# MLo7Ghinsan/GOOFER

Measured on AMD Instinct MI355X. Metric: resynth_frames_per_sec, higher is better.
Workload: dtype f32; 1 GPU; BASELINE config 3: 1024 notes/GPU x ~1.1 s, sr 44100, n_fft 1024, hop 256 (5.8 ms); per-note flags fa30fb-20fc10fd-10fw50fst40fsta20fstb-20fstc10fstd-10V80B20U-30 / fa-30fb20fc-10fd10fw-50fst-40fsta-20fstb20fstc-10fstd10V80B20U-30; one step = goofer_render_batch = goofer_assemble_batch + goofer_synth_batch (SillySampler.resample + gf.synthesize + V/B/U mix) from .goofy features and host-made plans; frames_per_gpu=194560, samples_per_gpu=49674240, sub_batches_per_gpu=1

## Files before the change

goofer_amd/csrc/api.hip:

```cpp
#include <math.h>
#include <stdarg.h>
#include <stdlib.h>

#include <algorithm>
#include <vector>

#include "common.h"
#include "launchers.h"

int goofer_fail(goofer_ctx *ctx, int code, const char *fmt, ...)
{
    if (ctx) {
        va_list ap;
        va_start(ap, fmt);
        vsnprintf(ctx->err, sizeof(ctx->err), fmt, ap);
        va_end(ap);
    }
    return code;
}

static goofer_ctx::kernel_state *kstate_of(goofer_ctx *ctx, const void *fn)
{
    for (int i = 0; i < ctx->n_kstate; ++i)
        if (ctx->kstate[i].fn == fn) return &ctx->kstate[i];
// ... 127 lines not shown
}

extern "C" {

const char *goofer_version(void) { return "goofer_hip 0.1 (gfx950)"; }

int goofer_create(int device_id, goofer_ctx **out)
{
    if (!out) return GOOFER_EINVAL;
    *out = nullptr;
    int count = 0;
    if (hipGetDeviceCount(&count) != hipSuccess || device_id < 0 || device_id >= count) return GOOFER_EHIP;
    if (hipSetDevice(device_id) != hipSuccess) return GOOFER_EHIP;
    goofer_ctx *c = new goofer_ctx();
    c->device = device_id;
    if (hipMalloc((void **)&c->ovf_flag, 64) != hipSuccess || hipMemset(c->ovf_flag, 0, 64) != hipSuccess) {
        delete c;
        return GOOFER_EHIP;
    }
    *out = c;
    return GOOFER_OK;
}

void goofer_destroy(goofer_ctx *ctx)
{
    if (!ctx) return;
    (void)hipSetDevice(ctx->device);
    (void)hipDeviceSynchronize();
    free_plan(ctx->plan);
    if (ctx->scratch) (void)hipFree(ctx->scratch);
    if (ctx->small) (void)hipFree(ctx->small);
// ... 218 lines not shown
    if (!ctx->ovf_flag) return GOOFER_OK;
    int32_t v = 0;
    HIP_TRY(ctx, hipMemcpy(&v, ctx->ovf_flag, sizeof(v), hipMemcpyDeviceToHost));
    if (v != 0) {
        HIP_TRY(ctx, hipMemset(ctx->ovf_flag, 0, sizeof(v)));
        return goofer_fail(ctx, GOOFER_EINVAL, "note %d of a batch since the last check has more pulse onsets than n / 2 + 16 (f0 above "
                           "sr / 2?): the pulses beyond its onset slots were dropped (the 'sg' layer's trackers have n + 16)", v - 1);
    }
    return GOOFER_OK;
}

int goofer_counter(goofer_ctx *ctx, const char *name, int64_t *value)
{
    if (!ctx || !name || !value) return GOOFER_EINVAL;
    int which = !strcmp(name, "pulse_fallback_notes") ? 1 : (!strcmp(name, "pulse_scanned_notes") ? 2 : -1);
    if (which < 0) return goofer_fail(ctx, GOOFER_EINVAL, "unknown counter %s", name);
    HIP_TRY(ctx, hipDeviceSynchronize());
    int32_t v = 0;
    HIP_TRY(ctx, hipMemcpy(&v, ctx->ovf_flag + which, sizeof(v), hipMemcpyDeviceToHost));
    *value = (int64_t)(uint32_t)v;
    return GOOFER_OK;
}

int64_t goofer_debug_fetch(goofer_ctx *ctx, int which, void *host_out, int64_t capacity_bytes)
{
    if (!ctx || which < 0 || which >= 16 || !ctx->dbg_ptr[which]) return GOOFER_EINVAL;
    if (int rc = goofer_check(ctx)) return rc;
    size_t nb = ctx->dbg_bytes[which] < (size_t)capacity_bytes ? ctx->dbg_bytes[which] : (size_t)capacity_bytes;
    if (hipMemcpy(host_out, ctx->dbg_ptr[which], nb, hipMemcpyDeviceToHost) != hipSuccess) return GOOFER_EHIP;
    return (int64_t)ctx->dbg_bytes[which];
}

// ... 73 lines not shown
    if (ctx && ctx->prof_stems) return PROF_NAMES_STEMS[stage];
    return (ctx && ctx->ola_fused) ? PROF_NAMES_OLA[stage] : PROF_NAMES[stage];
}

int goofer_set_option(goofer_ctx *ctx, const char *name, int value)
{
    if (!ctx || !name) return GOOFER_EINVAL;
    if (!strcmp(name, "fused_ola")) { ctx->ola_fused = value != 0; return GOOFER_OK; }
    if (!strcmp(name, "overlap")) { ctx->overlap = value != 0; return GOOFER_OK; }
    if (!strcmp(name, "stems")) { ctx->stems = value != 0; return GOOFER_OK; }
    if (!strcmp(name, "prof_only")) { ctx->prof_only = value < 0 || value >= PROF_STAGES ? -1 : value; return GOOFER_OK; }
    if (!strcmp(name, "skip_zero")) { ctx->skip_zero = value != 0; return GOOFER_OK; }
    if (!strcmp(name, "td_blur")) { ctx->td_blur = value != 0; return GOOFER_OK; }
    if (!strcmp(name, "pulse_scan")) { ctx->pulse_scan = value < 0 ? 0 : (value > 2 ? 2 : value); return GOOFER_OK; }
    if (!strcmp(name, "sa_fast")) { ctx->sa_fast = value != 0; return GOOFER_OK; }
    if (!strcmp(name, "value_f64")) { ctx->value_f64 = value != 0; return GOOFER_OK; }
    return goofer_fail(ctx, GOOFER_EINVAL, "unknown option %s", name);
}

int goofer_sizeof(int which)
{
    switch (which) {
    case 0: return (int)sizeof(goofer_note_params);
    case 1: return (int)sizeof(goofer_batch);
    case 2: return (int)sizeof(goofer_note_plan);
    case 3: return (int)sizeof(goofer_assembly);
    case 4: return (int)sizeof(goofer_onepole_job);
    case 5: return (int)sizeof(goofer_post_note);
    case 6: return (int)sizeof(goofer_post);
    case 7: return (int)sizeof(goofer_plan_request);
// ... 266 lines not shown
    if (!mask || !sample_off || !out || n_notes <= 0) return goofer_fail(ctx, GOOFER_EINVAL, "null argument");
    hipStream_t st = (hipStream_t)stream;
    std::vector<double> taps;
    int radius;
    gauss_taps_host(std::max(1.0, (double)sigma / 4.0), taps, radius);
    if (radius > 2048) return goofer_fail(ctx, GOOFER_EINVAL, "transition sigma too large");
    const size_t n_short = (size_t)(total_samples / 4 + n_notes + 16);
    int rc = grow_block(ctx, &ctx->small, &ctx->small_bytes, (taps.size() + 16 + n_short + 2 * (size_t)n_notes + 16) * sizeof(double),
                        "small block");
    if (rc) return rc;
    double *d_taps = (double *)ctx->small, *short_s = d_taps + taps.size() + 16, *steps = short_s + n_short;
    HIP_TRY(ctx, hipMemcpyAsync(d_taps, taps.data(), taps.size() * sizeof(double), hipMemcpyHostToDevice, st));
    HIP_TRY(ctx, hipStreamSynchronize(st));
    double acc = 0.0;
    for (double tv : taps) acc += tv * 1.0;
    if ((rc = launch_mask_short(ctx, mask, sample_off, n_notes, total_samples, d_taps, radius, acc, short_s, st))) return rc;
    return launch_mask_upsample(ctx, short_s, sample_off, n_notes, total_samples, steps, fast_interp != 0, out, st);
}

int goofer_normal_fill(goofer_ctx *ctx, uint64_t seed, const goofer_note_params *params, const int64_t *sample_off, int n_notes,
                       int64_t total_samples, int stream_tag, const unsigned char *note_on, const double *growl_scale, double *out,
                       void *stream)
{
    if (!ctx) return GOOFER_EINVAL;
    if (!params || !sample_off || !out) return goofer_fail(ctx, GOOFER_EINVAL, "goofer_normal_fill: null pointer");
    if (n_notes < 0 || total_samples < 0)
        return goofer_fail(ctx, GOOFER_EINVAL, "goofer_normal_fill: negative count (%d notes, %lld samples)", n_notes, (long long)total_samples);
    if (stream_tag < 0 || stream_tag > 4) return goofer_fail(ctx, GOOFER_EINVAL, "goofer_normal_fill: stream tag %d outside 0..4", stream_tag);
    if ((uintptr_t)out & 15) return goofer_fail(ctx, GOOFER_EINVAL, "goofer_normal_fill: out must be 16-byte aligned");
    return launch_normal_fill(ctx, seed, params, sample_off, n_notes, total_samples, stream_tag, note_on, growl_scale, out, (hipStream_t)stream);
}
// ... 86 lines not shown
```

goofer_amd/csrc/assemble.hip:

```cpp
#include <hip/hip_fp16.h>

#include <type_traits>

#include "binops_core.h"
#include "launchers.h"

constexpr int A_ROWS = 4;
constexpr int ES_HALO = 64;

__device__ __forceinline__ float exp_split(float x)
{
    const float L2E = 0x1.715476p+0f, L2E_LO = 0x1.4ae0c0p-26f, LN2 = 0x1.62e430p-1f;
    const float hi = x * L2E;
    float lo = __builtin_fmaf(x, L2E, -hi);
    lo = __builtin_fmaf(x, L2E_LO, lo);
    const float r = __builtin_amdgcn_exp2f(hi);
    return __builtin_fmaf(r, lo * LN2, r);
}

template <bool V64, int CH>
__global__ __launch_bounds__(256) void k_env_edit(const goofer_assembly a, int64_t total_edit_rows, const int *__restrict__ row_note)
{
    using acc_t = std::conditional_t<V64, double, float>;
    extern __shared__ __align__(16) unsigned char smem[];
// ... 641 lines not shown
}

__constant__ double EXP2_C[12] = {2.5678435993488206e-11, 4.4455382718708116e-10, 7.054911620801123e-09, 1.01780860092397e-07,
                                         1.321548679014431e-06,  1.5252733804059841e-05, 0.0001540353039338161,  0.0013333558146428443,
                                         0.009618129107628477,   0.05550410866482158,    0.24022650695910072,    0.6931471805599453};
__device__ __forceinline__ double exp2_poly(double x)
{
    const double n = rint(x), f = x - n;
    double q = EXP2_C[0];
#pragma unroll
    for (int k = 1; k < 12; ++k) q = fma(q, f, EXP2_C[k]);
    q = fma(q, f, 1.0);
    return ldexp(q, (int)n);
}

__device__ __forceinline__ void sample_assemble_one(const goofer_assembly &a, const goofer_note_plan &p, int64_t g)
{
    const int i = (int)(g - p.out_sample_off);
    const float *m = a.mask_src + p.src_sample_off;
    const float rd_tail = __builtin_amdgcn_rcpf((float)p.tail_len);

    double mk;
    if (p.vel_active) {
        const double pos = i < p.pre_new ? (double)i / p.vel_factor : (double)(i - p.pre_new) + (double)p.n_pre;
        const int n1 = p.n_before_vel;
        int j = pos >= 2147483647.0 ? n1 - 1 : (int)floor(pos);
        if (j > n1 - 1) j = n1 - 1;
        if (j < 0) j = 0;
        if (j >= n1 - 1) {
            mk = mask_stage1(m, p, n1 - 1, rd_tail);
        } else {
// ... 24 lines not shown
        } else if (j > 0 && x0 > tsec) {
            --j;
            x1 = x0;
            x0 = (double)j * dt;
        }
        if (j >= p.n_bend - 1) {
            midi = bend[p.n_bend - 1];
        } else {
            const double y0 = bend[j], y1 = bend[j + 1];
            const double den = x1 - x0;
            const double rden = fma(fma(-den, rdt, 1.0), rdt, rdt);
            midi = tsec == x0 ? y0 : ((y1 - y0) * rden) * (tsec - x0) + y0;
        }
    }
    const double hz = 440.0 * exp2_poly(div_by(midi - 69.0, 12.0, 0.083333333333333329));
    a.mask_out[g] = (float)mk;
    double f0 = mk * hz;
    if (p.pd_on && a.bend_out) a.bend_out[g] = (float)(midi - p.pd_base);
    if (p.fry_dir != 0) {
        const double base_hz = p.fry_hz * (mk > 0.0 ? 1.0 : 0.0);
        if (i >= p.fry_const_lo && i < p.fry_const_hi) {
            f0 = base_hz;
        } else if (i >= p.fry_glide_lo && i < p.fry_glide_hi) {
            const int m = p.fry_glide_hi - p.fry_glide_lo, k = i - p.fry_glide_lo;
            const double w = p.fry_dir > 0 ? ramp_up(k, m) : ramp_down(k, m);
            f0 = (1.0 - w) * base_hz + w * f0;
        }
    }
    a.f0_out[g] = (float)f0;
    if (a.f0_mul_out) a.f0_mul_out[g] = (float)(f0 * a.f0_mul[g]);
}


template <int SA_SPT>
__device__ __forceinline__ void sample_assemble_fast(const goofer_assembly &a, const goofer_note_plan &p, int64_t g0, int64_t total_samples)
{
    const float *__restrict__ m = a.mask_src + p.src_sample_off;
    const double *__restrict__ bend = a.bend + p.bend_off;
    float *__restrict__ mask_out = a.mask_out;
    float *__restrict__ f0_out = a.f0_out;
    const int n_pre = p.n_pre, s_pre = p.s_pre, s_tail = p.s_tail, tail_len = p.tail_len, ylen1 = (int)p.ylen - 1, nb1 = p.n_bend - 1;
    const bool tile = tail_len < p.want_samples, rev = p.reverse != 0, fv = p.force_voiced != 0;
    const float rd_tail = __builtin_amdgcn_rcpf((float)tail_len);
    const double sr = (double)a.sr, rsr = 1.0 / sr;
    const double dt = p.tick_dt, t_last = (double)nb1 * dt, rdt = fast_rcp(dt);
    const int64_t nbase = p.out_sample_off;
    int midx[SA_SPT], ja[SA_SPT], jb[SA_SPT];
    double tsec[SA_SPT], x0[SA_SPT], x1[SA_SPT];
    bool live[SA_SPT];
#pragma unroll
// ... 26 lines not shown
#pragma unroll
    for (int u = 0; u < SA_SPT; ++u) {
        mv[u] = fv ? 1.0f : m[midx[u]];
        y0[u] = bend[ja[u]];
        y1[u] = bend[jb[u]];
    }
    float fo[SA_SPT];
#pragma unroll
    for (int u = 0; u < SA_SPT; ++u) {
        const double den = x1[u] - x0[u];
        const double rden = fma(fma(-den, rdt, 1.0), rdt, rdt);
        const double midi = (ja[u] == jb[u] || tsec[u] == x0[u]) ? y0[u] : ((y1[u] - y0[u]) * rden) * (tsec[u] - x0[u]) + y0[u];
        const double hz = 440.0 * exp2_poly(div_by(midi - 69.0, 12.0, 0.083333333333333329));
        fo[u] = (float)((double)mv[u] * hz);
    }
#pragma unroll
    for (int u = 0; u < SA_SPT; ++u) {
        const int64_t g = g0 + threadIdx.x + (int64_t)u * blockDim.x;
        if (live[u]) {
            mask_out[g] = mv[u];
            f0_out[g] = fo[u];
        }
    }
}

template <int SA_SPT>
__global__ __launch_bounds__(256) void k_sample_assemble(const goofer_assembly a, int64_t total_samples, int fast)
{
    __shared__ int s_pair[2];
    const int64_t g0 = (int64_t)blockIdx.x * (blockDim.x * SA_SPT);
    if (threadIdx.x < WAVE) {
        auto key = [&](int k) { return a.notes[k].out_sample_off; };
        int64_t gl = g0 + (int64_t)blockDim.x * SA_SPT - 1;
        if (gl > total_samples - 1) gl = total_samples - 1;
        const int lo = wave_find(a.n_notes, g0, (int)threadIdx.x, key);
        const int hi = wave_find(a.n_notes, gl, (int)threadIdx.x, key);
        if (threadIdx.x == 0) { s_pair[0] = lo; s_pair[1] = hi; }
    }
    __syncthreads();
    const int n_lo = __builtin_amdgcn_readfirstlane(s_pair[0]), n_hi = __builtin_amdgcn_readfirstlane(s_pair[1]);
    if (n_lo == n_hi) {
        const goofer_note_plan &p = a.notes[n_lo];
        if (fast && !p.vel_active && p.fry_dir == 0 && !(p.pd_on && a.bend_out) && !a.f0_mul_out && p.n_out < (1 << 21) && p.tail_len < (1 << 24) &&
            p.tail_len > 0 && p.n_bend >= 1) {
            sample_assemble_fast<SA_SPT>(a, p, g0, total_samples);
            return;
        }
#pragma unroll
        for (int u = 0; u < SA_SPT; ++u) {
            const int64_t g = g0 + threadIdx.x + (int64_t)u * blockDim.x;
            if (g < total_samples) sample_assemble_one(a, p, g);
        }
    } else {
        for (int u = 0; u < SA_SPT; ++u) {
            const int64_t g = g0 + threadIdx.x + (int64_t)u * blockDim.x;
            if (g >= total_samples) break;
            int note = n_lo;
            while (note + 1 < a.n_notes && a.notes[note + 1].out_sample_off <= g) ++note;
            sample_assemble_one(a, a.notes[note], g);
        }
    }
}

__global__ __launch_bounds__(256) void k_env_fry(const goofer_assembly a, int64_t total_out_rows, const int *__restrict__ row_note, int hop)
{
    extern __shared__ __align__(16) unsigned char smem[];
    const int B = a.n_bins;
    const int wave = threadIdx.x >> 6, lane = threadIdx.x & 63;
    const int64_t orow = (int64_t)blockIdx.x * A_ROWS + wave;
    if (orow >= total_out_rows) return;
    const int note = row_note[orow];
    const goofer_note_plan p = a.notes[note];
    if (p.fry_a >= p.fry_b || p.n_out <= 0) return;
    const int64_t j = orow - p.env_off;
    int64_t c = j * hop + hop / 2;
// ... 46 lines not shown
        ctx->prof_asm_mask[ctx->prof_asm_steps] = 0;
    }
    auto mark = [&](int which, int edge, hipStream_t s) -> hipError_t {
        if (!pq || !(ctx->prof_only < 0 || ctx->prof_only == PROF_ASM0 + which)) return hipSuccess;
        if (edge) ctx->prof_asm_mask[ctx->prof_asm_steps] |= (unsigned char)(1u << which);
        return hipEventRecord(pq[2 * which + edge], s);
    };
    if (a->total_samples > 0) {
        const bool on_side = link.fork_early && ctx->ev_f0 && ctx->side && !a->any_fry;
        hipStream_t fst = on_side ? ctx->side : st;
        if (on_side) HIP_TRY(ctx, hipStreamWaitEvent(ctx->side, ctx->ev_entry, 0));
        constexpr int spt = 4;
        const dim3 sgrid((unsigned)((a->total_samples + 256 * spt - 1) / (256 * spt)));
        const int sa_fast = ctx->sa_fast ? 1 : 0;
        HIP_TRY(ctx, mark(2, 0, fst));
        hipLaunchKernelGGL(k_sample_assemble<spt>, sgrid, dim3(256), 0, fst, *a, a->total_samples, sa_fast);
        LAUNCH_CHECK(ctx);
        HIP_TRY(ctx, mark(2, 1, fst));
        if (link.fork_early && ctx->ev_f0) {
            HIP_TRY(ctx, hipEventRecord(ctx->ev_f0, fst));
            link.f0_ready = a->f0_out;
            link.f0_side = on_side;
        }
    }
    {
        const int64_t rows = std::max(a->total_edit_rows, a->total_out_rows);
        if (rows > 0) {
            hipLaunchKernelGGL(k_row_notes2, dim3((unsigned)((rows + 255) / 256)), dim3(256), 0, st, a->notes, a->n_notes, a->total_edit_rows,
                               a->total_out_rows, row_note_edit, row_note_out);
            LAUNCH_CHECK(ctx);
        }
// ... 74 lines not shown
```

goofer_amd/csrc/common.h:

```cpp
#pragma once

#include <hip/hip_runtime.h>
#include <stdint.h>
#include <stdio.h>
#include <string.h>

#include <vector>

#include "../../include/goofer_hip.h"

#define WAVE 64
#define PROF_STAGES 18
#define PROF_ASM0 15
#define PP_SPT 8
#define PULSE_TILE_INTS(samples) (4 * (((samples) + 256 * PP_SPT - 1) / (256 * PP_SPT)) + 64)
#define KN_K0 32
#define KN_DK 16
#define KN_KMAX 192
#define KN_CAND ((KN_KMAX - KN_K0) / KN_DK + 1)
#define KN_BINS_TOTAL (KN_CAND * KN_K0 + KN_DK * KN_CAND * (KN_CAND - 1) / 2)
#define PULSE_TAB_MAX 8192

struct lf_model {
    double ra = 0.02, rg = 1.7, rk = 0.8;
};
#define PULSE_PEAK_FLOATS (8193 + 1 + 6)

struct goofer_plan_t {
// ... 22 lines not shown
    float taps5_f[5] = {0}, taps175_f[15] = {0};
};

struct event_pool {
    int per_step;
    hipEvent_t *ev = nullptr;
    int steps = 0;
    hipEvent_t *step(int k) const { return ev + (size_t)k * per_step; }
};

struct render_link {
    bool fork_early = false;
    float *warp_dst = nullptr;
    const double *formants = nullptr;
    const goofer_note_params *params = nullptr;
    const float *f0_ready = nullptr;
    bool f0_side = false;
    bool warped = false;
};

struct goofer_ctx {
    int device = 0;
    char err[512] = {0};
    goofer_plan_t plan;
    void *scratch = nullptr;
    size_t scratch_bytes = 0;
    void *asm_scratch = nullptr;
    size_t asm_bytes = 0;
    void *small = nullptr;
    size_t small_bytes = 0;
    const void *dbg_ptr[16] = {nullptr};
    size_t dbg_bytes[16] = {0};
    bool overlap = true;
// ... 2 lines not shown
    hipEvent_t ev_entry = nullptr, ev_f0 = nullptr, ev_f0s = nullptr;
    int32_t *ovf_flag = nullptr;
    float *warp_rows = nullptr;
    size_t warp_rows_bytes = 0;
    event_pool prof_side{4};
    event_pool prof_main2{2};
    event_pool prof_asm{6};
    unsigned char prof_asm_mask[4096] = {0};
    int prof_asm_steps = 0;
    bool prof_side_used = false;
    bool ola_fused = true;
    bool stems = true;
    bool skip_zero = true;
    bool td_blur = true;
    bool prof_stems = false;
    bool sa_fast = true;
    bool value_f64 = false;
    int pulse_scan = 1;
    struct kernel_state {
        const void *fn;
        size_t lds;
        int waves;
        bool max_lds_set;
    } kstate[32] = {};
    int n_kstate = 0;
    bool prof_on = false;
    int prof_only = -1;
    int prof_steps = 0, prof_cap = 0;
    event_pool prof_ev{PROF_STAGES + 1};
    double *mask_taps = nullptr;
// ... 205 lines not shown
```

goofer_amd/csrc/launchers.h:

```cpp
#pragma once

#include "common.h"
#include "ragged.h"

struct onset_t;

int launch_gauss_rows64(goofer_ctx *ctx, const float *in, int ld, double *out, int ld64, int64_t rows, int n_bins, const double *d_taps,
                        int radius, hipStream_t st);
int launch_knot_error(goofer_ctx *ctx, const double *env2, int ld64, const int64_t *probe, int n_probe, int n_bins, const int *knot_bin,
                      int K, const int *lerp_idx, const float *w0, const float *w1, unsigned long long *err_bits, hipStream_t st);
int launch_knot_gather(goofer_ctx *ctx, const double *env2, int ld64, int64_t rows, const int *knot_bin, int K, uint16_t *knots,
                       hipStream_t st);
int launch_env_rows_fused(goofer_ctx *ctx, const float2 *S, int ldc, int64_t rows, int n_bins, const double *taps_env, int r_env,
                          const double *taps_fit, int r_fit, double *env_rows, int ld64, double *env2, int ld2, hipStream_t st);
int launch_knot_search(goofer_ctx *ctx, const double *env2, int ld2, const int64_t *probe_row, const int *probe_sig, int n_probe,
                       int n_bins, const int *knot_bin, const int *lerp_idx, const float *w0, const float *w1, unsigned long long *err_bits,
                       hipStream_t st);
int launch_knot_pick(goofer_ctx *ctx, const double *env2, int ld2, int64_t rows, const int *frame_sig, const int64_t *frame_off,
                     const int *knot_bin, const unsigned long long *err_bits, uint16_t *knots, int32_t *K_out, hipStream_t st);

size_t env_row_rec_bytes();
int launch_assemble(goofer_ctx *ctx, const goofer_assembly *a, int *row_note_edit, int *row_note_out, void *row_recs, render_link &link,
                    hipStream_t st);

// ... 92 lines not shown
                      const int *frame_note, const int64_t *frame_off, const int64_t *sample_off, int n_notes, const double *short_s,
                      double *steps, const goofer_note_params *params, float *harm, float *uv, float *bre, const unsigned char *frame_skip,
                      hipStream_t st);
int launch_frame_skip(goofer_ctx *ctx, const double *short_s, int64_t short_count, const int64_t *sample_off, const int64_t *frame_off,
                      const int *frame_note, int n_notes, int64_t total_frames, unsigned char *knot_eq, unsigned char *hop_flat,
                      unsigned char *frame_skip, hipStream_t st);
int launch_mask_upsample(goofer_ctx *ctx, const double *short_s, const int64_t *sample_off, int n_notes, int64_t total_samples,
                         double *steps, bool fast, float *out, hipStream_t st);
int launch_irfft_ola3(goofer_ctx *ctx, const float2 *S_h, const float2 *S_u, const float2 *S_b, int ldc, int64_t total_frames,
                      const int *frame_note, const int64_t *frame_off, const int64_t *sample_off, int n_notes, const float *note_mag,
                      const double *short_s, double *steps, const goofer_note_params *params, float *harm, float *uv, float *bre,
                      float *note_peak, hipStream_t st);
int launch_stem_peak(goofer_ctx *ctx, const float *harm, const float *uv, const float *bre, const int64_t *sample_off, int n_notes,
                     int64_t total, float *note_peak, hipStream_t st);
int launch_mask_short(goofer_ctx *ctx, const float *mask, const int64_t *sample_off, int n_notes, int64_t total_samples,
                      const double *d_taps, int radius, double tap_sum, double *short_s, hipStream_t st);
int launch_apply_gain(goofer_ctx *ctx, float *harm, float *uv, float *bre, float *rec, float *mix, const int64_t *sample_off, int n_notes,
                      int64_t total_samples, const goofer_note_params *params, const float *note_peak, bool write_stems, hipStream_t st);
int launch_ola3_gains(goofer_ctx *ctx, const float *fr_h, const float *fr_u, const float *fr_b, const float *note_mag,
                      const double *short_s, const int64_t *sample_off, const int64_t *frame_off, int n_notes, int64_t total_samples,
                      const goofer_note_params *params, double *steps, float *harm, float *uv, float *bre, float *note_peak,
                      hipStream_t st);

bool stems_supported(const goofer_plan_t &p);
int launch_frame_picks(goofer_ctx *ctx, const int64_t *frame_off, const int *frame_note, int64_t F, const int64_t *sample_off,
                       const float *f0, const float *mask, float2 *picks, hipStream_t st);
int launch_noise_stems(goofer_ctx *ctx, const float *env, int ld, const int64_t *row_src, const float *phi, int64_t F,
                       const int *frame_note, const int64_t *frame_off, const int64_t *sample_off, const float2 *picks,
                       const goofer_note_params *params, uint64_t seed, bool preblurred, const double *short_s, const double *steps,
                       float *uv, float *bre, unsigned char *hopz, hipStream_t st);
int launch_harm_stem(goofer_ctx *ctx, const float *pulse, const float *env, const float *env_plain, bool have_formants, int ld,
// ... 6 lines not shown
```

goofer_amd/csrc/samples.hip:

```cpp
#include <type_traits>
#include "fft_core.h"

#include "samples_core.h"
#include "launchers.h"

#define MS_MAXWIN 1152
#define MS_TILE 1024

__global__ __launch_bounds__(256) void k_mask_short(const float *__restrict__ mask, const int64_t *__restrict__ sample_off,
                                                    int n_notes, int64_t total_short, const double *__restrict__ taps, int radius,
                                                    double *__restrict__ short_s, double tap_sum)
{
    extern __shared__ __align__(16) unsigned char smem[];
    double *s_taps = reinterpret_cast<double *>(smem);
    float *s_all = reinterpret_cast<float *>(s_taps + (2 * radius + 1));
    __shared__ int s_lo[2];
    for (int i = threadIdx.x; i < 2 * radius + 1; i += blockDim.x) s_taps[i] = taps[i];
    const int64_t g0 = (int64_t)blockIdx.x * MS_TILE;
    int64_t g1 = g0 + MS_TILE;
    if (g1 > total_short) g1 = total_short;
    if (threadIdx.x < WAVE) {
        auto key = [&](int k) { return short_base(sample_off, k); };
        const int a = wave_find(n_notes, g0, (int)threadIdx.x, key);
        const int b = wave_find(n_notes, g1 - 1, (int)threadIdx.x, key);
        if (threadIdx.x == 0) { s_lo[0] = a; s_lo[1] = b; }
    }
    __syncthreads();
    const int lane = threadIdx.x & 63, wv = threadIdx.x >> 6;
    const int n_lo = __builtin_amdgcn_readfirstlane(s_lo[0]), n_hi = __builtin_amdgcn_readfirstlane(s_lo[1]);

    if (2 * radius + MS_TILE <= 4 * MS_MAXWIN) {
        for (int note = n_lo; note <= n_hi; ++note) {
            const int64_t sb = short_base(sample_off, note);
            const int64_t base = sample_off[note], n = sample_off[note + 1] - base;
            const int64_t ns = (n + MASK_DS - 1) / MASK_DS;
            const int64_t s0 = g0 > sb ? g0 : sb, s1 = g1 < sb + ns ? g1 : sb + ns;
            if (s1 <= s0) continue;
            const int64_t q0 = s0 - sb;
            const int len = (int)(s1 - s0);
            const float *m = mask + base;
            if (note != n_lo) __syncthreads();
            for (int w = threadIdx.x; w < len + 2 * radius; w += blockDim.x) s_all[w] = m[MASK_DS * reflect_index(q0 - radius + w, ns)];
            __syncthreads();
            for (int c0 = wv * WAVE; c0 < len; c0 += 4 * WAVE) {
                const float *x0 = s_all + c0;
                const int cl = len - c0 < WAVE ? len - c0 : WAVE;
                const bool live = lane < cl;
                bool all0 = true, all1 = true;
                for (int w = lane; w < cl + 2 * radius; w += WAVE) {
                    const float v = x0[w];
                    all0 &= v == 0.0f;
                    all1 &= v == 1.0f;
                }
                double acc;
                if (__all(all0)) {
                    acc = 0.0;
                } else if (__all(all1)) {
                    acc = tap_sum;
                } else {
                    acc = 0.0;
                    const float *x = x0 + lane;
                    if (live)
                        for (int j = 0; j <= 2 * radius; ++j) acc += s_taps[j] * (double)x[j];
                }
                if (live) short_s[s0 + c0 + lane] = acc;
            }
        }
        return;
    }
    for (int64_t g = g0 + threadIdx.x; g < g1; g += blockDim.x) {
        int note = n_lo;
        while (note + 1 < n_notes && short_base(sample_off, note + 1) <= g) ++note;
        const int64_t q = g - short_base(sample_off, note);
        const int64_t base = sample_off[note], n = sample_off[note + 1] - base;
        const int64_t ns = (n + MASK_DS - 1) / MASK_DS;
        if (q >= ns) continue;
        const float *m = mask + base;
        double acc = 0.0;
// ... 840 lines not shown
{
    const sample_tile<> t(sample_off, n_notes, total);
    const int64_t g = t.g;
    const float pk = t.live ? fabsf((harm[g] + uv[g]) + bre[g]) : 0.f;
    const int note = t.live && !t.uniform() ? t.note(sample_off) : t.lo;
    note_reduce(t, note, t.live, pk, [](float a, float b) { return fmaxf(a, b); }, [&](int k, float m) { atomic_max_pos(note_peak + k, m); });
}

int launch_stem_peak(goofer_ctx *ctx, const float *harm, const float *uv, const float *bre, const int64_t *sample_off, int n_notes,
                     int64_t total, float *note_peak, hipStream_t st)
{
    return launch_per_sample(ctx, k_stem_peak, total, 256, 0, st, harm, uv, bre, sample_off, n_notes, total, note_peak);
}

int launch_mask_short(goofer_ctx *ctx, const float *mask, const int64_t *sample_off, int n_notes, int64_t total_samples,
                      const double *d_taps, int radius, double tap_sum, double *short_s, hipStream_t st)
{
    int64_t total_short = total_samples / MASK_DS + n_notes;
    if (total_short <= 0) return GOOFER_OK;
    hipLaunchKernelGGL(k_mask_short, dim3((unsigned)((total_short + MS_TILE - 1) / MS_TILE)), dim3(256),
                       sizeof(double) * (2 * radius + 1) + sizeof(float) * 4 * MS_MAXWIN, st, mask, sample_off, n_notes, total_short,
                       d_taps, radius, short_s, tap_sum);
    LAUNCH_CHECK(ctx);
    return GOOFER_OK;
}

int launch_apply_gain(goofer_ctx *ctx, float *harm, float *uv, float *bre, float *rec, float *mix, const int64_t *sample_off,
                      int n_notes, int64_t total_samples, const goofer_note_params *params, const float *note_peak, bool write_stems,
                      hipStream_t st)
{
    return launch_per_sample(ctx, k_apply_gain, total_samples, 256 * SPT, 0, st, harm, uv, bre, rec, mix, sample_off, n_notes, total_samples,
                             params, note_peak, write_stems ? 1 : 0);
}

int launch_ola3_gains(goofer_ctx *ctx, const float *fr_h, const float *fr_u, const float *fr_b, const float *note_mag,
                      const double *short_s, const int64_t *sample_off, const int64_t *frame_off, int n_notes, int64_t total_samples,
                      const goofer_note_params *params, double *steps, float *harm, float *uv, float *bre, float *note_peak,
// ... 10 lines not shown
```

goofer_amd/csrc/synth.hip:

```cpp
#include <algorithm>
#include <vector>

#include "common.h"
#include "launchers.h"
#include "samples_core.h"

__device__ __forceinline__ void frame_pick_and_row(int64_t f, int note, const int64_t *__restrict__ frame_off,
                                                   const int64_t *__restrict__ env_off, int64_t *__restrict__ row_src,
                                                   const int64_t *__restrict__ sample_off, const float *__restrict__ f0,
                                                   const float *__restrict__ mask, int hop, float2 *__restrict__ picks)
{
    int64_t t = f - frame_off[note];
    if (picks) {
        const int64_t base = sample_off[note], n = sample_off[note + 1] - base;
        float2 pv = make_float2(0.f, 0.f);
        if (n > 0) {
            int64_t at = t * hop;
            if (at >= n) at = ((n - 1) / hop) * hop;
            pv = make_float2(f0[base + at], mask[base + at]);
        }
        picks[f] = pv;
    }
    const int64_t rows = env_off[note + 1] - env_off[note];
    if (t > rows - 1) t = rows - 1;
// ... 205 lines not shown
};

struct synth_call {
    goofer_ctx *ctx;
    const goofer_batch *b;
    const render_link &link;
    const synth_route &r;
    synth_scratch &s;
    stage_clock &clk;
    hipStream_t st;
    int64_t F, N;
    int n;

    int mask_short() const
    {
        return launch_mask_short(ctx, b->mask, b->sample_off, n, N, ctx->mask_taps, ctx->mask_taps_radius, ctx->mask_taps_sum, s.short_s, st);
    }
    int late_picks() const
    {
        return r.picks_on ? GOOFER_OK : launch_frame_picks(ctx, b->frame_off, s.frame_note, F, b->sample_off, s.f0s, b->mask, s.picks, st);
    }
    int noise_walker() const
    {
        return launch_noise_stems(ctx, b->env_noise ? b->env_noise : b->env, b->ld, s.row_src, b->phi, F, s.frame_note, b->frame_off,
                                  b->sample_off, s.picks, b->params, b->seed, b->env_noise != nullptr, s.short_s, s.note_steps, b->uv,
                                  b->bre, s.hopz, st);
    }
    int noise_spectra() const
    {
        return launch_noise_spectra(ctx, s.S_uv, s.S_br, spec_stride(ctx->plan.n_bins), F, s.frame_note, b->frame_off, b->sample_off, s.f0s,
                                    b->mask, b->env_noise ? b->env_noise : b->env, b->phi, b->ld, b->params, b->seed, s.row_src,
// ... 89 lines not shown
            return rc;
        return clk.close();
    }
};

static int assemble_batch(goofer_ctx *ctx, const goofer_assembly *asmb, render_link &link, hipStream_t st)
{
    if (asmb->n_notes <= 0) return GOOFER_OK;
    if (asmb->ld < asmb->n_bins || asmb->max_K < 2 || asmb->max_K > 4096) return goofer_fail(ctx, GOOFER_EINVAL, "bad assembly geometry");
    if (asmb->n_bins > 1025) return goofer_fail(ctx, GOOFER_EINVAL, "the resampler's assembly takes n_fft <= 2048 (%d bins)", asmb->n_bins);
    if (asmb->any_fry && ctx->plan.hop <= 0) return goofer_fail(ctx, GOOFER_EINVAL, "the fry envelope warp needs goofer_plan first");
    goofer_assembly a = *asmb;
    int *map_edit;
    float *edit_rows;
    char *recs;
    int rc = carve_block(ctx, &ctx->asm_scratch, &ctx->asm_bytes, "assembly scratch", [&](arena &m) {
        map_edit = m.take<int>((size_t)(a.total_edit_rows + a.total_out_rows) + 64);
        edit_rows = m.take<float>(a.edit_rows ? 0 : (size_t)a.total_edit_rows * a.ld);
        recs = m.take<char>((size_t)a.total_out_rows * env_row_rec_bytes());
    });
    if (rc) return rc;
    if (!a.edit_rows) a.edit_rows = edit_rows;
    return launch_assemble(ctx, &a, map_edit, map_edit + a.total_edit_rows, recs, link, st);
}

static int synth_batch(goofer_ctx *ctx, const goofer_batch *b, render_link &link, hipStream_t st)
{
    const goofer_plan_t &p = ctx->plan;
    if (b->n_bins != p.n_bins || b->ld < p.n_bins) return goofer_fail(ctx, GOOFER_EINVAL, "batch geometry does not match the plan");
    if (b->n_notes <= 0 || b->total_samples <= 0) return GOOFER_OK;
    const int64_t F = b->total_frames, N = b->total_samples;
    const int n = b->n_notes;
    const synth_route r = synth_route_of(ctx, b, link);
    synth_scratch s;
    int rc = carve_scratch(ctx, [&](arena &a) { carve_synth(a, p, r, F, N, n, b->ld, s); });
    if (rc) return rc;
// ... 174 lines not shown
    if (ctx->overlap && asmb->f0_out == b->f0 && asmb->n_notes > 0) {
        if ((rc = ensure_side_stream(ctx))) return rc;
        HIP_TRY(ctx, hipEventRecord(ctx->ev_entry, st));
        link.fork_early = true;
    }
    if (synth_route_of(ctx, b, link).walkers && ctx->overlap && asmb->env_out == b->env && asmb->n_notes == b->n_notes &&
        asmb->total_out_rows == b->total_env_rows && asmb->ld == b->ld && !asmb->any_fry) {
        const size_t need = (size_t)b->total_env_rows * b->ld * sizeof(float);
        if (need > ctx->warp_rows_bytes &&
            (rc = grow_block(ctx, (void **)&ctx->warp_rows, &ctx->warp_rows_bytes, need + need / 4, "warped rows")))
            return rc;
        link.formants = b->formants;
        link.params = b->params;
        link.warp_dst = ctx->warp_rows;
    }
    rc = assemble_batch(ctx, asmb, link, st);
    if (!rc) rc = synth_batch(ctx, b, link, st);
    if (link.f0_side) (void)hipStreamWaitEvent(st, ctx->ev_f0, 0);
    return rc;
}

}
```

Measured before the change: 106.2 million frames/s.

## Emit per-tile mask flatness flags in sample assembly to skip mask_short staging

```diff
diff --git a/goofer_amd/csrc/api.hip b/goofer_amd/csrc/api.hip
--- a/goofer_amd/csrc/api.hip
+++ b/goofer_amd/csrc/api.hip
@@ -165,7 +165,7 @@
     if (hipSetDevice(device_id) != hipSuccess) return GOOFER_EHIP;
     goofer_ctx *c = new goofer_ctx();
     c->device = device_id;
-    if (hipMalloc((void **)&c->ovf_flag, 64) != hipSuccess || hipMemset(c->ovf_flag, 0, 64) != hipSuccess) {
+    if (hipMalloc((void **)&c->ovf_flag, OVF_WORDS * sizeof(int32_t)) != hipSuccess || hipMemset(c->ovf_flag, 0, OVF_WORDS * sizeof(int32_t)) != hipSuccess) {
         delete c;
         return GOOFER_EHIP;
     }
@@ -414,8 +414,18 @@
 {
     if (!ctx || !name || !value) return GOOFER_EINVAL;
     int which = !strcmp(name, "pulse_fallback_notes") ? 1 : (!strcmp(name, "pulse_scanned_notes") ? 2 : -1);
-    if (which < 0) return goofer_fail(ctx, GOOFER_EINVAL, "unknown counter %s", name);
+    const int mask_c = !strcmp(name, "mask_flag_segments") ? 0 : (!strcmp(name, "mask_staged_segments") ? 1 : -1);
+    if (which < 0 && mask_c < 0) return goofer_fail(ctx, GOOFER_EINVAL, "unknown counter %s", name);
     HIP_TRY(ctx, hipDeviceSynchronize());
+    if (mask_c >= 0) {
+        static_assert(OVF_WORDS <= 8192, "goofer_counter reads the words through a stack buffer");
+        int32_t w[OVF_WORDS];
+        HIP_TRY(ctx, hipMemcpy(w, ctx->ovf_flag, sizeof(w), hipMemcpyDeviceToHost));
+        int64_t sum = 0;
+        for (int sl = 0; sl < MASK_COUNTER_SLOTS; ++sl) sum += (int64_t)(uint32_t)w[MASK_COUNTERS + (2 * sl + mask_c) * MASK_COUNTER_STRIDE];
+        *value = sum;
+        return GOOFER_OK;
+    }
     int32_t v = 0;
     HIP_TRY(ctx, hipMemcpy(&v, ctx->ovf_flag + which, sizeof(v), hipMemcpyDeviceToHost));
     *value = (int64_t)(uint32_t)v;
@@ -519,6 +529,7 @@
     if (!strcmp(name, "td_blur")) { ctx->td_blur = value != 0; return GOOFER_OK; }
     if (!strcmp(name, "pulse_scan")) { ctx->pulse_scan = value < 0 ? 0 : (value > 2 ? 2 : value); return GOOFER_OK; }
     if (!strcmp(name, "sa_fast")) { ctx->sa_fast = value != 0; return GOOFER_OK; }
+    if (!strcmp(name, "mask_flags")) { ctx->mask_flags = value != 0; return GOOFER_OK; }
     if (!strcmp(name, "value_f64")) { ctx->value_f64 = value != 0; return GOOFER_OK; }
     return goofer_fail(ctx, GOOFER_EINVAL, "unknown option %s", name);
 }
@@ -815,7 +826,7 @@
     HIP_TRY(ctx, hipStreamSynchronize(st));
     double acc = 0.0;
     for (double tv : taps) acc += tv * 1.0;
-    if ((rc = launch_mask_short(ctx, mask, sample_off, n_notes, total_samples, d_taps, radius, acc, short_s, st))) return rc;
+    if ((rc = launch_mask_short(ctx, mask, sample_off, n_notes, total_samples, d_taps, radius, acc, short_s, nullptr, nullptr, st))) return rc;
     return launch_mask_upsample(ctx, short_s, sample_off, n_notes, total_samples, steps, fast_interp != 0, out, st);
 }
 
diff --git a/goofer_amd/csrc/assemble.hip b/goofer_amd/csrc/assemble.hip
--- a/goofer_amd/csrc/assemble.hip
+++ b/goofer_amd/csrc/assemble.hip
@@ -679,7 +679,7 @@
     return ldexp(q, (int)n);
 }
 
-__device__ __forceinline__ void sample_assemble_one(const goofer_assembly &a, const goofer_note_plan &p, int64_t g)
+__device__ __forceinline__ float sample_assemble_one(const goofer_assembly &a, const goofer_note_plan &p, int64_t g)
 {
     const int i = (int)(g - p.out_sample_off);
     const float *m = a.mask_src + p.src_sample_off;
@@ -734,7 +734,8 @@
         }
     }
     const double hz = 440.0 * exp2_poly(div_by(midi - 69.0, 12.0, 0.083333333333333329));
-    a.mask_out[g] = (float)mk;
+    const float mk_f = (float)mk;
+    a.mask_out[g] = mk_f;
     double f0 = mk * hz;
     if (p.pd_on && a.bend_out) a.bend_out[g] = (float)(midi - p.pd_base);
     if (p.fry_dir != 0) {
@@ -749,11 +750,21 @@
     }
     a.f0_out[g] = (float)f0;
     if (a.f0_mul_out) a.f0_mul_out[g] = (float)(f0 * a.f0_mul[g]);
-}
-
-
-template <int SA_SPT>
-__device__ __forceinline__ void sample_assemble_fast(const goofer_assembly &a, const goofer_note_plan &p, int64_t g0, int64_t total_samples)
+    return mk_f;
+}
+
+
+__device__ __forceinline__ unsigned mask_vote(float mk) { return (mk == 0.0f ? 0u : 1u) | (mk == 1.0f ? 0u : 2u); }
+
+struct sa_kernarg {
+    goofer_assembly a;
+    int64_t total_samples;
+    int fast;
+    unsigned char *tile_flags;
+};
+template <int SA_SPT, bool FLAGS>
+__device__ __forceinline__ void sample_assemble_fast(const goofer_assembly &a, const goofer_note_plan &p, int64_t g0, int64_t total_samples,
+                                                     unsigned &bad, unsigned char *&flag_dst)
 {
     const float *__restrict__ m = a.mask_src + p.src_sample_off;
     const double *__restrict__ bend = a.bend + p.bend_off;
@@ -810,6 +821,10 @@
         const double hz = 440.0 * exp2_poly(div_by(midi - 69.0, 12.0, 0.083333333333333329));
         fo[u] = (float)((double)mv[u] * hz);
     }
+    if (FLAGS) {
+        asm volatile("" : "+v"(fo[SA_SPT - 1]));
+        flag_dst = COLD(sa_kernarg, tile_flags);
+    }
 #pragma unroll
     for (int u = 0; u < SA_SPT; ++u) {
         const int64_t g = g0 + threadIdx.x + (int64_t)u * blockDim.x;
@@ -818,10 +833,13 @@
             f0_out[g] = fo[u];
         }
     }
-}
-
-template <int SA_SPT>
-__global__ __launch_bounds__(256) void k_sample_assemble(const goofer_assembly a, int64_t total_samples, int fast)
+#pragma unroll
+    for (int u = 0; u < SA_SPT; ++u)
+        if (live[u]) bad |= mask_vote(mv[u]);
+}
+
+template <int SA_SPT, bool FLAGS>
+__global__ __launch_bounds__(256) void k_sample_assemble(const goofer_assembly a, int64_t total_samples, int fast, unsigned char *__restrict__ tile_flags)
 {
     __shared__ int s_pair[2];
     const int64_t g0 = (int64_t)blockIdx.x * (blockDim.x * SA_SPT);
@@ -835,17 +853,20 @@
     }
     __syncthreads();
     const int n_lo = __builtin_amdgcn_readfirstlane(s_pair[0]), n_hi = __builtin_amdgcn_readfirstlane(s_pair[1]);
+    unsigned bad = 0u;
+    unsigned char *flag_dst = nullptr;
+    auto vote = [&](float mk) { bad |= mask_vote(mk); };
     if (n_lo == n_hi) {
         const goofer_note_plan &p = a.notes[n_lo];
         if (fast && !p.vel_active && p.fry_dir == 0 && !(p.pd_on && a.bend_out) && !a.f0_mul_out && p.n_out < (1 << 21) && p.tail_len < (1 << 24) &&
             p.tail_len > 0 && p.n_bend >= 1) {
-            sample_assemble_fast<SA_SPT>(a, p, g0, total_samples);
-            return;
-        }
-#pragma unroll
-        for (int u = 0; u < SA_SPT; ++u) {
-            const int64_t g = g0 + threadIdx.x + (int64_t)u * blockDim.x;
-            if (g < total_samples) sample_assemble_one(a, p, g);
+            sample_assemble_fast<SA_SPT, FLAGS>(a, p, g0, total_samples, bad, flag_dst);
+        } else {
+#pragma unroll
+            for (int u = 0; u < SA_SPT; ++u) {
+                const int64_t g = g0 + threadIdx.x + (int64_t)u * blockDim.x;
+                if (g < total_samples) vote(sample_assemble_one(a, p, g));
+            }
         }
     } else {
         for (int u = 0; u < SA_SPT; ++u) {
@@ -853,8 +874,13 @@
             if (g >= total_samples) break;
             int note = n_lo;
             while (note + 1 < a.n_notes && a.notes[note + 1].out_sample_off <= g) ++note;
-            sample_assemble_one(a, a.notes[note], g);
-        }
+            vote(sample_assemble_one(a, a.notes[note], g));
+        }
+    }
+    if (FLAGS) {
+        const int bits = (__any(bad & 1u) ? 1 : 0) | (__any(bad & 2u) ? 2 : 0);
+        if (!flag_dst) flag_dst = COLD(sa_kernarg, tile_flags);
+        if ((threadIdx.x & (WAVE - 1)) == 0) flag_dst[4 * (size_t)blockIdx.x + (threadIdx.x >> 6)] = (unsigned char)bits;
     }
 }
 
@@ -931,7 +957,13 @@
         const dim3 sgrid((unsigned)((a->total_samples + 256 * spt - 1) / (256 * spt)));
         const int sa_fast = ctx->sa_fast ? 1 : 0;
         HIP_TRY(ctx, mark(2, 0, fst));
-        hipLaunchKernelGGL(k_sample_assemble<spt>, sgrid, dim3(256), 0, fst, *a, a->total_samples, sa_fast);
+        static_assert(256 * spt == SA_TILE, "one tile-flag word per workgroup of k_sample_assemble");
+        if (link.tile_flags_dst) {
+            hipLaunchKernelGGL((k_sample_assemble<spt, true>), sgrid, dim3(256), 0, fst, *a, a->total_samples, sa_fast, link.tile_flags_dst);
+            link.tile_flags = link.tile_flags_dst;
+        } else {
+            hipLaunchKernelGGL((k_sample_assemble<spt, false>), sgrid, dim3(256), 0, fst, *a, a->total_samples, sa_fast, (unsigned char *)nullptr);
+        }
         LAUNCH_CHECK(ctx);
         HIP_TRY(ctx, mark(2, 1, fst));
         if (link.fork_early && ctx->ev_f0) {
diff --git a/goofer_amd/csrc/common.h b/goofer_amd/csrc/common.h
--- a/goofer_amd/csrc/common.h
+++ b/goofer_amd/csrc/common.h
@@ -12,6 +12,11 @@
 #define WAVE 64
 #define PROF_STAGES 18
 #define PROF_ASM0 15
+#define SA_TILE 1024
+#define MASK_COUNTERS 32
+#define MASK_COUNTER_SLOTS 64
+#define MASK_COUNTER_STRIDE 32
+#define OVF_WORDS (MASK_COUNTERS + 2 * MASK_COUNTER_SLOTS * MASK_COUNTER_STRIDE)
 #define PP_SPT 8
 #define PULSE_TILE_INTS(samples) (4 * (((samples) + 256 * PP_SPT - 1) / (256 * PP_SPT)) + 64)
 #define KN_K0 32
@@ -64,9 +69,12 @@
     float *warp_dst = nullptr;
     const double *formants = nullptr;
     const goofer_note_params *params = nullptr;
+    bool want_tile_flags = false;
+    unsigned char *tile_flags_dst = nullptr;
     const float *f0_ready = nullptr;
     bool f0_side = false;
     bool warped = false;
+    const unsigned char *tile_flags = nullptr;
 };
 
 struct goofer_ctx {
@@ -99,6 +107,7 @@
     bool skip_zero = true;
     bool td_blur = true;
     bool prof_stems = false;
+    bool mask_flags = true;
     bool sa_fast = true;
     bool value_f64 = false;
     int pulse_scan = 1;
diff --git a/goofer_amd/csrc/launchers.h b/goofer_amd/csrc/launchers.h
--- a/goofer_amd/csrc/launchers.h
+++ b/goofer_amd/csrc/launchers.h
@@ -130,7 +130,8 @@
 int launch_stem_peak(goofer_ctx *ctx, const float *harm, const float *uv, const float *bre, const int64_t *sample_off, int n_notes,
                      int64_t total, float *note_peak, hipStream_t st);
 int launch_mask_short(goofer_ctx *ctx, const float *mask, const int64_t *sample_off, int n_notes, int64_t total_samples,
-                      const double *d_taps, int radius, double tap_sum, double *short_s, hipStream_t st);
+                      const double *d_taps, int radius, double tap_sum, double *short_s, const unsigned char *tile_flags,
+                      int32_t *counters, hipStream_t st);
 int launch_apply_gain(goofer_ctx *ctx, float *harm, float *uv, float *bre, float *rec, float *mix, const int64_t *sample_off, int n_notes,
                       int64_t total_samples, const goofer_note_params *params, const float *note_peak, bool write_stems, hipStream_t st);
 int launch_ola3_gains(goofer_ctx *ctx, const float *fr_h, const float *fr_u, const float *fr_b, const float *note_mag,
diff --git a/goofer_amd/csrc/samples.hip b/goofer_amd/csrc/samples.hip
--- a/goofer_amd/csrc/samples.hip
+++ b/goofer_amd/csrc/samples.hip
@@ -6,10 +6,12 @@
 
 #define MS_MAXWIN 1152
 #define MS_TILE 1024
+#define MS_QUART (MS_TILE / 4)
 
 __global__ __launch_bounds__(256) void k_mask_short(const float *__restrict__ mask, const int64_t *__restrict__ sample_off,
                                                     int n_notes, int64_t total_short, const double *__restrict__ taps, int radius,
-                                                    double *__restrict__ short_s, double tap_sum)
+                                                    double *__restrict__ short_s, double tap_sum,
+                                                    const unsigned char *__restrict__ tile_flags, int32_t *__restrict__ counters)
 {
     extern __shared__ __align__(16) unsigned char smem[];
     double *s_taps = reinterpret_cast<double *>(smem);
@@ -30,6 +32,7 @@
     const int n_lo = __builtin_amdgcn_readfirstlane(s_lo[0]), n_hi = __builtin_amdgcn_readfirstlane(s_lo[1]);
 
     if (2 * radius + MS_TILE <= 4 * MS_MAXWIN) {
+        bool staged = false;
         for (int note = n_lo; note <= n_hi; ++note) {
             const int64_t sb = short_base(sample_off, note);
             const int64_t base = sample_off[note], n = sample_off[note + 1] - base;
@@ -39,29 +42,64 @@
             const int64_t q0 = s0 - sb;
             const int len = (int)(s1 - s0);
             const float *m = mask + base;
-            if (note != n_lo) __syncthreads();
-            for (int w = threadIdx.x; w < len + 2 * radius; w += blockDim.x) s_all[w] = m[MASK_DS * reflect_index(q0 - radius + w, ns)];
+            unsigned flat0 = 0u, flat1 = 0u;
+            const int nq = (len + MS_QUART - 1) / MS_QUART;
+            if (tile_flags) {
+                auto tile_of = [&](int64_t q) {
+                    q = q < 0 ? 0 : (q > ns - 1 ? ns - 1 : q);
+                    return (base + MASK_DS * q) / SA_TILE;
+                };
+                const int64_t t0 = tile_of(q0 - radius), t1 = tile_of(q0 + len - 1 + radius);
+                if (t1 - t0 < WAVE) {
+                    const uint32_t f = lane <= (int)(t1 - t0) ? reinterpret_cast<const uint32_t *>(tile_flags)[t0 + lane] : 0x03030303u;
+                    const uint64_t z = __ballot((f & 0x01010101u) == 0u), o = __ballot((f & 0x02020202u) == 0u);
+                    const int ql = (lane < nq ? lane : 0) * MS_QUART, qh = ql + MS_QUART < len ? ql + MS_QUART : len;
+                    const int a = (int)(tile_of(q0 + ql - radius) - t0), b = (int)(tile_of(q0 + qh - 1 + radius) - t0);
+                    const uint64_t need = (b - a >= 63 ? ~0ull : (1ull << (b - a + 1)) - 1ull) << a;
+                    const bool is0 = lane < nq && (z & need) == need, is1 = lane < nq && !is0 && (o & need) == need;
+                    flat0 = (unsigned)__ballot(is0);
+                    flat1 = (unsigned)__ballot(is1);
+                }
+            }
+            const unsigned flat = flat0 | flat1;
+            if (flat == (1u << nq) - 1u) {
+                for (int w = threadIdx.x; w < len; w += blockDim.x) short_s[s0 + w] = ((flat1 >> (w / MS_QUART)) & 1u) ? tap_sum : 0.0;
+                if (counters && threadIdx.x == 0) atomicAdd(counters + (2 * (blockIdx.x % MASK_COUNTER_SLOTS)) * MASK_COUNTER_STRIDE, 1);
+                continue;
+            }
+            if (counters && threadIdx.x == 0) atomicAdd(counters + (2 * (blockIdx.x % MASK_COUNTER_SLOTS) + 1) * MASK_COUNTER_STRIDE, 1);
+            if (staged) __syncthreads();
+            staged = true;
+            for (int w = threadIdx.x; w < len + 2 * radius; w += blockDim.x) {
+                bool want = flat == 0u;
+                for (int k = 0; k < nq && !want; ++k) want = !((flat >> k) & 1u) && w >= k * MS_QUART && w < (k + 1) * MS_QUART + 2 * radius;
+                if (want) s_all[w] = m[MASK_DS * reflect_index(q0 - radius + w, ns)];
+            }
             __syncthreads();
             for (int c0 = wv * WAVE; c0 < len; c0 += 4 * WAVE) {
                 const float *x0 = s_all + c0;
                 const int cl = len - c0 < WAVE ? len - c0 : WAVE;
                 const bool live = lane < cl;
-                bool all0 = true, all1 = true;
-                for (int w = lane; w < cl + 2 * radius; w += WAVE) {
-                    const float v = x0[w];
-                    all0 &= v == 0.0f;
-                    all1 &= v == 1.0f;
-                }
                 double acc;
-                if (__all(all0)) {
-                    acc = 0.0;
-                } else if (__all(all1)) {
-                    acc = tap_sum;
+                if ((flat >> (c0 / MS_QUART)) & 1u) {
+                    acc = ((flat1 >> (c0 / MS_QUART)) & 1u) ? tap_sum : 0.0;
                 } else {
-                    acc = 0.0;
-                    const float *x = x0 + lane;
-                    if (live)
-                        for (int j = 0; j <= 2 * radius; ++j) acc += s_taps[j] * (double)x[j];
+                    bool all0 = true, all1 = true;
+                    for (int w = lane; w < cl + 2 * radius; w += WAVE) {
+                        const float v = x0[w];
+                        all0 &= v == 0.0f;
+                        all1 &= v == 1.0f;
+                    }
+                    if (__all(all0)) {
+                        acc = 0.0;
+                    } else if (__all(all1)) {
+                        acc = tap_sum;
+                    } else {
+                        acc = 0.0;
+                        const float *x = x0 + lane;
+                        if (live)
+                            for (int j = 0; j <= 2 * radius; ++j) acc += s_taps[j] * (double)x[j];
+                    }
                 }
                 if (live) short_s[s0 + c0 + lane] = acc;
             }
@@ -932,13 +970,14 @@
 }
 
 int launch_mask_short(goofer_ctx *ctx, const float *mask, const int64_t *sample_off, int n_notes, int64_t total_samples,
-                      const double *d_taps, int radius, double tap_sum, double *short_s, hipStream_t st)
+                      const double *d_taps, int radius, double tap_sum, double *short_s, const unsigned char *tile_flags,
+                      int32_t *counters, hipStream_t st)
 {
     int64_t total_short = total_samples / MASK_DS + n_notes;
     if (total_short <= 0) return GOOFER_OK;
     hipLaunchKernelGGL(k_mask_short, dim3((unsigned)((total_short + MS_TILE - 1) / MS_TILE)), dim3(256),
                        sizeof(double) * (2 * radius + 1) + sizeof(float) * 4 * MS_MAXWIN, st, mask, sample_off, n_notes, total_short,
-                       d_taps, radius, short_s, tap_sum);
+                       d_taps, radius, short_s, tap_sum, tile_flags, counters);
     LAUNCH_CHECK(ctx);
     return GOOFER_OK;
 }
diff --git a/goofer_amd/csrc/synth.hip b/goofer_amd/csrc/synth.hip
--- a/goofer_amd/csrc/synth.hip
+++ b/goofer_amd/csrc/synth.hip
@@ -243,7 +243,8 @@
 
     int mask_short() const
     {
-        return launch_mask_short(ctx, b->mask, b->sample_off, n, N, ctx->mask_taps, ctx->mask_taps_radius, ctx->mask_taps_sum, s.short_s, st);
+        return launch_mask_short(ctx, b->mask, b->sample_off, n, N, ctx->mask_taps, ctx->mask_taps_radius, ctx->mask_taps_sum, s.short_s,
+                                 link.tile_flags, ctx->ovf_flag ? ctx->ovf_flag + MASK_COUNTERS : nullptr, st);
     }
     int late_picks() const
     {
@@ -363,12 +364,16 @@
     int *map_edit;
     float *edit_rows;
     char *recs;
+    unsigned char *flags;
+    const bool want_flags = link.want_tile_flags && a.mask_out && a.total_samples > 0;
     int rc = carve_block(ctx, &ctx->asm_scratch, &ctx->asm_bytes, "assembly scratch", [&](arena &m) {
         map_edit = m.take<int>((size_t)(a.total_edit_rows + a.total_out_rows) + 64);
         edit_rows = m.take<float>(a.edit_rows ? 0 : (size_t)a.total_edit_rows * a.ld);
         recs = m.take<char>((size_t)a.total_out_rows * env_row_rec_bytes());
+        flags = m.take<unsigned char>(want_flags ? 4 * (size_t)((a.total_samples + SA_TILE - 1) / SA_TILE) + 64 : 0);
     });
     if (rc) return rc;
+    link.tile_flags_dst = want_flags ? flags : nullptr;
     if (!a.edit_rows) a.edit_rows = edit_rows;
     return launch_assemble(ctx, &a, map_edit, map_edit + a.total_edit_rows, recs, link, st);
 }
@@ -573,6 +578,8 @@
         link.params = b->params;
         link.warp_dst = ctx->warp_rows;
     }
+    link.want_tile_flags = ctx->mask_flags && asmb->mask_out && asmb->mask_out == b->mask && asmb->total_samples == b->total_samples &&
+                           asmb->n_notes == b->n_notes;
     rc = assemble_batch(ctx, asmb, link, st);
     if (!rc) rc = synth_batch(ctx, b, link, st);
     if (link.f0_side) (void)hipStreamWaitEvent(st, ctx->ev_f0, 0);
```

Result: faster. 109.0 million frames/s, median of 6 (+2.6%).
